# luisdiaz1997/GPzoo

Hardware: AMD Instinct MI355X
Metric: ELBO evals/sec (L=32-latent evaluations, all GPUs) at M=2048 inducing, N=200000, L=32 latents/GPU x 1 GPU(s) (higher is better)
Workload: dtype f32; 1 GPU; BASELINE configs[2]: Slide-seq-shaped synthetic, N=200000 spots, M=2048, L=32 latents/GPU x 1 GPU(s), matern32, f32; latents_total=32, whitened=True, chunk=0, factor_dtype=f64

## Files before the change

### gpzoo_amd/csrc/kgrad.hip

```cpp
#include "kgrad.h"
#include "mmops.h"

namespace gpz {

__device__ __forceinline__ float kg_exp(float x) { return __builtin_amdgcn_exp2f(x * 1.44269504088896341f); }
__device__ __forceinline__ double kg_exp(double x) { return exp(x); }
__device__ __forceinline__ float kg_sqrt(float x) { return sqrtf(x); }
__device__ __forceinline__ double kg_sqrt(double x) { return sqrt(x); }
__device__ __forceinline__ float kg_rsqrt(float x) { return rsqrtf(x); }
__device__ __forceinline__ double kg_rsqrt(double x) { return 1.0 / sqrt(x); }
__device__ __forceinline__ float kg_pow(float x, float y) { return __builtin_amdgcn_exp2f(y * __builtin_amdgcn_logf(x)); }
__device__ __forceinline__ double kg_pow(double x, double y) { return pow(x, y); }

template <typename T, int KIND>
__global__ __launch_bounds__(256) void kgrad_kernel(KgradArgs a) {
  const int l = blockIdx.y, wave = threadIdx.x >> 6, lane = threadIdx.x & 63;
  const int64_t m = (int64_t)blockIdx.x * 4 + wave;
  if (m >= a.M) return;
  const T* kb = static_cast<const T*>(a.Kbar) + (int64_t)l * a.stride + m * a.ld;
  const T* Zp = static_cast<const T*>(a.Z);
  const T* Xp = static_cast<const T*>(a.X);
  const int d = a.d;
  const T sig = static_cast<const T*>(a.sigma)[l];
  const T ell = static_cast<const T*>(a.ell)[l];
  const T s2 = sig * sig, il2 = (T)1 / (ell * ell);
  T z[4] = {0, 0, 0, 0};
  for (int k = 0; k < d; ++k) z[k] = Zp[m * d + k];
  const int gz = (KIND == 2) ? ((uint64_t)a.gZ[m] < (uint64_t)a.G ? (int)a.gZ[m] : 0) : 0;
  const T aeff = (KIND == 2) ? static_cast<const T*>(a.ga)[l] : (T)0;
  const T gpow = (T)a.gpow;
  double dz[4] = {0, 0, 0, 0}, dsig = 0, dell = 0, da = 0;
  constexpr int UN = 4;
  for (int64_t c0 = lane; c0 < a.ncols; c0 += 64 * UN) {
    T g[UN], x[UN][4];
    int gx[UN];
#pragma unroll
    for (int u = 0; u < UN; ++u) {
      const int64_t c = c0 + 64 * u;
      const bool in = c < a.ncols;
      g[u] = in ? kb[c] : (T)0;
#pragma unroll
      for (int k = 0; k < 4; ++k) x[u][k] = (in && k < d) ? Xp[c * d + k] : (T)0;
      gx[u] = (KIND == 2 && in) ? ((uint64_t)a.gX[c] < (uint64_t)a.G ? (int)a.gX[c] : 0) : 0;
    }
    T pz[4] = {0, 0, 0, 0}, psig = 0, pell = 0, pa = 0;
#pragma unroll
    for (int u = 0; u < UN; ++u) {
      T diff[4], d2 = 0;
#pragma unroll
      for (int k = 0; k < 4; ++k) { diff[k] = (k < d) ? z[k] - x[u][k] : (T)0; d2 = fma(diff[k], diff[k], d2); }
      T cz;
      if (KIND == 0) {
        const T kv = s2 * kg_exp((T)-0.5 * d2 * il2);
        psig += g[u] * (T)2 * kv / sig;
        pell += g[u] * kv * d2 * il2 / ell;
        cz = -kv * il2;
      } else if (KIND == 1) {
        const T v = (T)1.7320508075688772935 * kg_sqrt(d2) / ell, e = kg_exp(-v);
        psig += g[u] * (T)2 * sig * ((T)1 + v) * e;
        pell += g[u] * s2 * v * v * e / ell;
        cz = -s2 * (T)3 * il2 * e;
      } else if (KIND == 4) {
        const T rr = kg_sqrt(d2), kv = s2 * kg_exp(-rr / ell);
        psig += g[u] * (T)2 * kv / sig;
        pell += g[u] * kv * rr * il2;
        cz = d2 > (T)0 ? -(kv / ell) * kg_rsqrt(d2) : (T)0;
      } else if (KIND == 5) {
        const T v = (T)2.2360679774997896964 * kg_sqrt(d2) / ell, e = kg_exp(-v), q3 = v * v / (T)3;
        psig += g[u] * (T)2 * sig * ((T)1 + v + q3) * e;
        pell += g[u] * s2 * q3 * ((T)1 + v) * e / ell;
        cz = -s2 * (T)5 / (T)3 * il2 * ((T)1 + v) * e;
      } else {
        const T r2 = static_cast<const T*>(a.gr2)[gz * a.G + gx[u]];
        const T den = aeff * r2 + (T)1;
        const T kv = s2 * kg_exp((T)-0.5 * d2 * il2 / den) * kg_pow(den, -gpow);
        psig += g[u] * (T)2 * kv / sig;
        pell += g[u] * kv * d2 * il2 / (ell * den);
        pa += g[u] * kv * ((T)0.5 * d2 * il2 / (den * den) - gpow / den) * r2;
        cz = -kv * il2 / den;
      }
      const T gc = g[u] * cz;
#pragma unroll
      for (int k = 0; k < 4; ++k) pz[k] = fma(gc, diff[k], pz[k]);
    }
    dsig += (double)psig; dell += (double)pell; da += (double)pa;
#pragma unroll
    for (int k = 0; k < 4; ++k) dz[k] += (double)pz[k];
  }
  double v[7] = {dz[0], dz[1], dz[2], dz[3], dsig * a.scalar_scale, dell * a.scalar_scale, da * a.scalar_scale};
#pragma unroll
  for (int i = 0; i < 7; ++i)
    for (int o = 32; o > 0; o >>= 1) v[i] += __shfl_down(v[i], o);
  if (lane == 0) {
    double* dst = a.acc + ((int64_t)l * a.Mp + m) * 8;
#pragma unroll
    for (int i = 0; i < 7; ++i) dst[i] += v[i];
  }
}

int kgrad_launch(int dtype, int kind, const KgradArgs& a, int L, hipStream_t s) {
  GPZ_REQUIRE((kind >= 0 && kind <= 2) || kind == GPZ_KERNEL_MATERN12 || kind == GPZ_KERNEL_MATERN52,
              "kgrad: unknown kernel kind %d", kind);
  dim3 grid((unsigned)((a.M + 3) / 4), (unsigned)L), block(256);
#define GPZ_KG(T, K) hipLaunchKernelGGL((kgrad_kernel<T, K>), grid, block, 0, s, a)
#define GPZ_KG_KINDS(T) \
  switch (kind) { case 0: GPZ_KG(T, 0); break; case 1: GPZ_KG(T, 1); break; case 4: GPZ_KG(T, 4); break; \
                  case 5: GPZ_KG(T, 5); break; default: GPZ_KG(T, 2); break; }
  if (dtype == GPZ_F32) GPZ_KG_KINDS(float) else GPZ_KG_KINDS(double)
#undef GPZ_KG_KINDS
#undef GPZ_KG
  GPZ_LAUNCH_OK();
  return 0;
}

}

extern "C" size_t gpz_kgrad_workspace_bytes(int64_t nA, int32_t n_latent) {
  if (nA < 1 || n_latent < 1) return 0;
  gpz::Carver c(nullptr);
  c.take<double>((int64_t)n_latent * nA * 8);
  return c.used();
}

extern "C" int gpz_kgrad(const gpz_kernel_desc* k, const void* A, int64_t nA, const void* B, int64_t nB, int32_t d,
                         const int64_t* gA, const int64_t* gB, const void* Kbar, int64_t ldk, int64_t stride_k,
                         double* grad_theta, double* grad_A, void* ws, size_t ws_bytes, void* stream) {
  using namespace gpz;
  GPZ_REQUIRE(k && A && B && Kbar && ws, "gpz_kgrad: null pointer");
  GPZ_REQUIRE(nA >= 1 && nB >= 1 && ldk >= nB && d >= 1 && d <= 4, "gpz_kgrad: bad extents nA=%lld nB=%lld ldk=%lld d=%d",
              (long long)nA, (long long)nB, (long long)ldk, d);
  GPZ_REQUIRE((k->kind >= 0 && k->kind <= 2) || k->kind == GPZ_KERNEL_MATERN12 || k->kind == GPZ_KERNEL_MATERN52,
              "gpz_kgrad: kernel kind %d has no parameters to differentiate", k->kind);
  GPZ_REQUIRE(k->n_latent >= 1 && (k->dtype == GPZ_F32 || k->dtype == GPZ_F64), "gpz_kgrad: bad kernel description");
  if (k->kind == GPZ_KERNEL_MGGP_RBF)
    GPZ_REQUIRE(gA && gB && k->group_a && k->group_r2 && k->n_groups >= 1, "gpz_kgrad: MGGP kernel needs groups, group_a, group_r2");
  GPZ_REQUIRE(ws_bytes >= gpz_kgrad_workspace_bytes(nA, k->n_latent), "gpz_kgrad: workspace too small");
  hipStream_t s = static_cast<hipStream_t>(stream);
  const int L = k->n_latent;
  Carver c(ws);
  double* acc = c.take<double>((int64_t)L * nA * 8);
  GPZ_HIP_OK(hipMemsetAsync(acc, 0, sizeof(double) * L * nA * 8, s));
  KgradArgs a;
  a.Kbar = Kbar; a.ld = ldk; a.stride = stride_k; a.Z = A; a.X = B; a.gZ = gA; a.gX = gB;
  a.sigma = k->sigma; a.ell = k->lengthscale; a.ga = k->group_a; a.gr2 = k->group_r2;
  a.gpow = k->group_pow; a.scalar_scale = 1.0; a.M = nA; a.ncols = nB; a.Mp = nA; a.d = d; a.G = k->n_groups; a.acc = acc;
  if (int rc = kgrad_launch(k->dtype, k->kind, a, L, s)) return rc;
  return kgrad_finish(acc, L, nA, nA, d, nullptr, grad_A, grad_theta, s);
}
```

Baseline: 2.654 ELBO evals/s.

## Restructure kgrad kernel: two rows per wave, factored sums, vector loads, templated dim

Each wavefront now handles two inducing rows and reuses every loaded X column for both. Columns are read as 4-wide vector loads, and the input dimension becomes a template parameter. The per-element math is rewritten to accumulate a few kernel-specific moment sums (e, e*r, e*d2, ...) with sigma, lengthscale and constants folded into the exponent scale, and the gradients are rebuilt in double once per row at the end. This is meant to cut redundant X loads, per-element divides and multiplies, and wasted lanes when d<4. In exchange it adds register pressure and many more template instantiations, and the vector loads assume 16-byte-friendly alignment of Kbar rows.

```diff
diff --git a/gpzoo_amd/csrc/kgrad.hip b/gpzoo_amd/csrc/kgrad.hip
--- a/gpzoo_amd/csrc/kgrad.hip
+++ b/gpzoo_amd/csrc/kgrad.hip
@@ -3,111 +3,216 @@
 
 namespace gpz {
 
-__device__ __forceinline__ float kg_exp(float x) { return __builtin_amdgcn_exp2f(x * 1.44269504088896341f); }
-__device__ __forceinline__ double kg_exp(double x) { return exp(x); }
-__device__ __forceinline__ float kg_sqrt(float x) { return sqrtf(x); }
-__device__ __forceinline__ double kg_sqrt(double x) { return sqrt(x); }
-__device__ __forceinline__ float kg_rsqrt(float x) { return rsqrtf(x); }
-__device__ __forceinline__ double kg_rsqrt(double x) { return 1.0 / sqrt(x); }
-__device__ __forceinline__ float kg_pow(float x, float y) { return __builtin_amdgcn_exp2f(y * __builtin_amdgcn_logf(x)); }
-__device__ __forceinline__ double kg_pow(double x, double y) { return pow(x, y); }
-
-template <typename T, int KIND>
+constexpr int KG_ROWS = 2;
+
+template <typename T> struct KgMath;
+template <> struct KgMath<float> {
+  typedef float vec4 __attribute__((ext_vector_type(4), aligned(4)));
+  static constexpr float escale = 1.44269504088896341f;
+  static __device__ __forceinline__ float exps(float x) { return __builtin_amdgcn_exp2f(x); }
+  static __device__ __forceinline__ float sqrt(float x) { return __builtin_amdgcn_sqrtf(x); }
+  static __device__ __forceinline__ float rsqrt(float x) { return rsqrtf(x); }
+  static __device__ __forceinline__ float rcp(float x) { return __builtin_amdgcn_rcpf(x); }
+  static __device__ __forceinline__ float pow(float x, float y) { return __builtin_amdgcn_exp2f(y * __builtin_amdgcn_logf(x)); }
+};
+template <> struct KgMath<double> {
+  typedef double vec4 __attribute__((ext_vector_type(4), aligned(8)));
+  static constexpr double escale = 1.0;
+  static __device__ __forceinline__ double exps(double x) { return ::exp(x); }
+  static __device__ __forceinline__ double sqrt(double x) { return ::sqrt(x); }
+  static __device__ __forceinline__ double rsqrt(double x) { return 1.0 / ::sqrt(x); }
+  static __device__ __forceinline__ double rcp(double x) { return 1.0 / x; }
+  static __device__ __forceinline__ double pow(double x, double y) { return ::pow(x, y); }
+};
+
+__host__ __device__ constexpr int kg_nsums(int kind) { return kind == 0 ? 2 : kind == 1 ? 3 : kind == 4 ? 2 : 4; }
+
+template <typename T> struct KgConst { T c2, c1, aeff, gpow; };
+
+template <typename T, bool FULL>
+__device__ __forceinline__ void kg_load4(const T* p, int64_t c, int64_t n, T (&o)[4]) {
+  if (FULL) {
+    const typename KgMath<T>::vec4 q = *reinterpret_cast<const typename KgMath<T>::vec4*>(p + c);
+    o[0] = q.x; o[1] = q.y; o[2] = q.z; o[3] = q.w;
+  } else {
+#pragma unroll
+    for (int j = 0; j < 4; ++j) o[j] = c + j < n ? p[c + j] : (T)0;
+  }
+}
+
+template <typename T, int D, int R> struct KgTrip { T g[R][4], x[4 * D]; int gx[4]; };
+
+template <typename T, int KIND, int D, int R, bool FULL>
+__device__ __forceinline__ void kg_load(const KgradArgs& a, const T* (&kb)[R], const T* Xp, int64_t c,
+                                        KgTrip<T, D, R>& t) {
+#pragma unroll
+  for (int r = 0; r < R; ++r) kg_load4<T, FULL>(kb[r], c, a.ncols, t.g[r]);
+#pragma unroll
+  for (int q = 0; q < D; ++q) {
+    T o[4];
+    kg_load4<T, FULL>(Xp, c * D + 4 * q, a.ncols * D, o);
+#pragma unroll
+    for (int j = 0; j < 4; ++j) t.x[4 * q + j] = o[j];
+  }
+#pragma unroll
+  for (int j = 0; j < 4; ++j)
+    t.gx[j] = (KIND == 2 && (FULL || c + j < a.ncols)) ? ((uint64_t)a.gX[c + j] < (uint64_t)a.G ? (int)a.gX[c + j] : 0) : 0;
+}
+
+template <typename T, int KIND, int D, int R>
+__device__ __forceinline__ void kg_accum(const KgradArgs& a, const KgConst<T>& k, const T (&z)[R][D], const int (&gz)[R],
+                                         const KgTrip<T, D, R>& t, T (&S)[R][kg_nsums(KIND) + D]) {
+  using Mth = KgMath<T>;
+  constexpr int NS = kg_nsums(KIND);
+#pragma unroll
+  for (int j = 0; j < 4; ++j)
+#pragma unroll
+    for (int r = 0; r < R; ++r) {
+      T diff[D];
+      diff[0] = z[r][0] - t.x[j * D];
+      T d2 = diff[0] * diff[0];
+#pragma unroll
+      for (int q = 1; q < D; ++q) { diff[q] = z[r][q] - t.x[j * D + q]; d2 = fma(diff[q], diff[q], d2); }
+      const T g = t.g[r][j];
+      T w;
+      if (KIND == 0) {
+        const T e = g * Mth::exps(d2 * k.c2);
+        S[r][0] += e; S[r][1] = fma(e, d2, S[r][1]);
+        w = e;
+      } else if (KIND == 1) {
+        const T rr = Mth::sqrt(d2), e = g * Mth::exps(rr * k.c2);
+        S[r][0] += e; S[r][1] = fma(e, rr, S[r][1]); S[r][2] = fma(e, d2, S[r][2]);
+        w = e;
+      } else if (KIND == 4) {
+        const T ri = d2 > (T)0 ? Mth::rsqrt(d2) : (T)0, rr = d2 * ri, e = g * Mth::exps(rr * k.c2);
+        S[r][0] += e; S[r][1] = fma(e, rr, S[r][1]);
+        w = e * ri;
+      } else if (KIND == 5) {
+        const T rr = Mth::sqrt(d2), e = g * Mth::exps(rr * k.c2), er = e * rr;
+        S[r][0] += e; S[r][1] += er; S[r][2] = fma(e, d2, S[r][2]); S[r][3] = fma(er, d2, S[r][3]);
+        w = fma(er, k.c1, e);
+      } else {
+        const T r2 = static_cast<const T*>(a.gr2)[gz[r] * a.G + t.gx[j]];
+        const T den = fma(k.aeff, r2, (T)1), id = Mth::rcp(den);
+        const T e = g * Mth::exps(d2 * k.c2 * id) * Mth::pow(den, -k.gpow), u = e * id, ur = u * r2;
+        S[r][0] += e; S[r][1] = fma(u, d2, S[r][1]); S[r][2] = fma(ur * id, d2, S[r][2]); S[r][3] += ur;
+        w = u;
+      }
+#pragma unroll
+      for (int q = 0; q < D; ++q) S[r][NS + q] = fma(w, diff[q], S[r][NS + q]);
+    }
+}
+
+template <int KIND, int D>
+__device__ __forceinline__ void kg_finish_row(const double* v, double sig, double ell, double gpow, double scale, double* dst) {
+  constexpr int NS = kg_nsums(KIND);
+  const double il = 1.0 / ell, s2 = sig * sig, il2 = il * il;
+  double dsig, dell, da = 0, fz;
+  if (KIND == 0) {
+    dsig = 2 * sig * v[0]; dell = s2 * il2 * il * v[1]; fz = -s2 * il2;
+  } else if (KIND == 1) {
+    const double c1 = 1.7320508075688772935 * il;
+    dsig = 2 * sig * (v[0] + c1 * v[1]); dell = s2 * il * c1 * c1 * v[2]; fz = -3 * s2 * il2;
+  } else if (KIND == 4) {
+    dsig = 2 * sig * v[0]; dell = s2 * il2 * v[1]; fz = -s2 * il;
+  } else if (KIND == 5) {
+    const double c1 = 2.2360679774997896964 * il, q = c1 * c1 / 3;
+    dsig = 2 * sig * (v[0] + c1 * v[1] + q * v[2]); dell = s2 * il * q * (v[2] + c1 * v[3]); fz = -(5.0 / 3.0) * s2 * il2;
+  } else {
+    dsig = 2 * sig * v[0]; dell = s2 * il2 * il * v[1]; da = s2 * (0.5 * il2 * v[2] - gpow * v[3]); fz = -s2 * il2;
+  }
+#pragma unroll
+  for (int q = 0; q < D; ++q) dst[q] += fz * v[NS + q];
+  dst[4] += dsig * scale; dst[5] += dell * scale;
+  if (KIND == 2) dst[6] += da * scale;
+}
+
+template <typename T, int KIND, int D>
 __global__ __launch_bounds__(256) void kgrad_kernel(KgradArgs a) {
+  constexpr int R = KG_ROWS, NS = kg_nsums(KIND), NV = NS + D;
+  using Mth = KgMath<T>;
   const int l = blockIdx.y, wave = threadIdx.x >> 6, lane = threadIdx.x & 63;
-  const int64_t m = (int64_t)blockIdx.x * 4 + wave;
-  if (m >= a.M) return;
-  const T* kb = static_cast<const T*>(a.Kbar) + (int64_t)l * a.stride + m * a.ld;
+  const int64_t m0 = ((int64_t)blockIdx.x * 4 + wave) * R;
+  if (m0 >= a.M) return;
   const T* Zp = static_cast<const T*>(a.Z);
   const T* Xp = static_cast<const T*>(a.X);
-  const int d = a.d;
+  const T* kbl = static_cast<const T*>(a.Kbar) + (int64_t)l * a.stride;
   const T sig = static_cast<const T*>(a.sigma)[l];
   const T ell = static_cast<const T*>(a.ell)[l];
-  const T s2 = sig * sig, il2 = (T)1 / (ell * ell);
-  T z[4] = {0, 0, 0, 0};
-  for (int k = 0; k < d; ++k) z[k] = Zp[m * d + k];
-  const int gz = (KIND == 2) ? ((uint64_t)a.gZ[m] < (uint64_t)a.G ? (int)a.gZ[m] : 0) : 0;
-  const T aeff = (KIND == 2) ? static_cast<const T*>(a.ga)[l] : (T)0;
-  const T gpow = (T)a.gpow;
-  double dz[4] = {0, 0, 0, 0}, dsig = 0, dell = 0, da = 0;
-  constexpr int UN = 4;
-  for (int64_t c0 = lane; c0 < a.ncols; c0 += 64 * UN) {
-    T g[UN], x[UN][4];
-    int gx[UN];
-#pragma unroll
-    for (int u = 0; u < UN; ++u) {
-      const int64_t c = c0 + 64 * u;
-      const bool in = c < a.ncols;
-      g[u] = in ? kb[c] : (T)0;
-#pragma unroll
-      for (int k = 0; k < 4; ++k) x[u][k] = (in && k < d) ? Xp[c * d + k] : (T)0;
-      gx[u] = (KIND == 2 && in) ? ((uint64_t)a.gX[c] < (uint64_t)a.G ? (int)a.gX[c] : 0) : 0;
-    }
-    T pz[4] = {0, 0, 0, 0}, psig = 0, pell = 0, pa = 0;
-#pragma unroll
-    for (int u = 0; u < UN; ++u) {
-      T diff[4], d2 = 0;
-#pragma unroll
-      for (int k = 0; k < 4; ++k) { diff[k] = (k < d) ? z[k] - x[u][k] : (T)0; d2 = fma(diff[k], diff[k], d2); }
-      T cz;
-      if (KIND == 0) {
-        const T kv = s2 * kg_exp((T)-0.5 * d2 * il2);
-        psig += g[u] * (T)2 * kv / sig;
-        pell += g[u] * kv * d2 * il2 / ell;
-        cz = -kv * il2;
-      } else if (KIND == 1) {
-        const T v = (T)1.7320508075688772935 * kg_sqrt(d2) / ell, e = kg_exp(-v);
-        psig += g[u] * (T)2 * sig * ((T)1 + v) * e;
-        pell += g[u] * s2 * v * v * e / ell;
-        cz = -s2 * (T)3 * il2 * e;
-      } else if (KIND == 4) {
-        const T rr = kg_sqrt(d2), kv = s2 * kg_exp(-rr / ell);
-        psig += g[u] * (T)2 * kv / sig;
-        pell += g[u] * kv * rr * il2;
-        cz = d2 > (T)0 ? -(kv / ell) * kg_rsqrt(d2) : (T)0;
-      } else if (KIND == 5) {
-        const T v = (T)2.2360679774997896964 * kg_sqrt(d2) / ell, e = kg_exp(-v), q3 = v * v / (T)3;
-        psig += g[u] * (T)2 * sig * ((T)1 + v + q3) * e;
-        pell += g[u] * s2 * q3 * ((T)1 + v) * e / ell;
-        cz = -s2 * (T)5 / (T)3 * il2 * ((T)1 + v) * e;
-      } else {
-        const T r2 = static_cast<const T*>(a.gr2)[gz * a.G + gx[u]];
-        const T den = aeff * r2 + (T)1;
-        const T kv = s2 * kg_exp((T)-0.5 * d2 * il2 / den) * kg_pow(den, -gpow);
-        psig += g[u] * (T)2 * kv / sig;
-        pell += g[u] * kv * d2 * il2 / (ell * den);
-        pa += g[u] * kv * ((T)0.5 * d2 * il2 / (den * den) - gpow / den) * r2;
-        cz = -kv * il2 / den;
-      }
-      const T gc = g[u] * cz;
-#pragma unroll
-      for (int k = 0; k < 4; ++k) pz[k] = fma(gc, diff[k], pz[k]);
-    }
-    dsig += (double)psig; dell += (double)pell; da += (double)pa;
-#pragma unroll
-    for (int k = 0; k < 4; ++k) dz[k] += (double)pz[k];
-  }
-  double v[7] = {dz[0], dz[1], dz[2], dz[3], dsig * a.scalar_scale, dell * a.scalar_scale, da * a.scalar_scale};
-#pragma unroll
-  for (int i = 0; i < 7; ++i)
-    for (int o = 32; o > 0; o >>= 1) v[i] += __shfl_down(v[i], o);
+  const T il = (T)1 / ell;
+  KgConst<T> k;
+  k.c1 = (T)2.2360679774997896964 * il;
+  k.c2 = (KIND == 1 ? (T)-1.7320508075688772935 * il : KIND == 4 ? -il : KIND == 5 ? -k.c1 : (T)-0.5 * il * il) * Mth::escale;
+  k.aeff = (KIND == 2) ? static_cast<const T*>(a.ga)[l] : (T)0;
+  k.gpow = (T)a.gpow;
+  const T* kb[R];
+  T z[R][D];
+  int gz[R];
+#pragma unroll
+  for (int r = 0; r < R; ++r) {
+    const int64_t m = m0 + r < a.M ? m0 + r : a.M - 1;
+    kb[r] = kbl + m * a.ld;
+#pragma unroll
+    for (int q = 0; q < D; ++q) z[r][q] = Zp[m * D + q];
+    gz[r] = (KIND == 2) ? ((uint64_t)a.gZ[m] < (uint64_t)a.G ? (int)a.gZ[m] : 0) : 0;
+  }
+  T S[R][NV];
+  double tot[R][NV];
+#pragma unroll
+  for (int r = 0; r < R; ++r)
+#pragma unroll
+    for (int i = 0; i < NV; ++i) { S[r][i] = 0; tot[r][i] = 0; }
+  auto fold = [&]() {
+#pragma unroll
+    for (int r = 0; r < R; ++r)
+#pragma unroll
+      for (int i = 0; i < NV; ++i) { tot[r][i] += (double)S[r][i]; S[r][i] = 0; }
+  };
+  const int64_t nfull = a.ncols / 512;
+  for (int64_t it = 0; it < nfull; ++it) {
+    const int64_t c = it * 512 + lane * 4;
+    KgTrip<T, D, R> t0, t1;
+    kg_load<T, KIND, D, R, true>(a, kb, Xp, c, t0);
+    kg_load<T, KIND, D, R, true>(a, kb, Xp, c + 256, t1);
+    kg_accum<T, KIND, D, R>(a, k, z, gz, t0, S);
+    kg_accum<T, KIND, D, R>(a, k, z, gz, t1, S);
+    fold();
+  }
+  for (int64_t c0 = nfull * 512; c0 < a.ncols; c0 += 256) {
+    KgTrip<T, D, R> t;
+    kg_load<T, KIND, D, R, false>(a, kb, Xp, c0 + lane * 4, t);
+    kg_accum<T, KIND, D, R>(a, k, z, gz, t, S);
+  }
+  fold();
+#pragma unroll
+  for (int r = 0; r < R; ++r)
+#pragma unroll
+    for (int i = 0; i < NV; ++i)
+      for (int o = 32; o > 0; o >>= 1) tot[r][i] += __shfl_down(tot[r][i], o);
   if (lane == 0) {
-    double* dst = a.acc + ((int64_t)l * a.Mp + m) * 8;
-#pragma unroll
-    for (int i = 0; i < 7; ++i) dst[i] += v[i];
+#pragma unroll
+    for (int r = 0; r < R; ++r)
+      if (m0 + r < a.M)
+        kg_finish_row<KIND, D>(tot[r], (double)sig, (double)ell, a.gpow, a.scalar_scale,
+                               a.acc + ((int64_t)l * a.Mp + m0 + r) * 8);
   }
 }
 
 int kgrad_launch(int dtype, int kind, const KgradArgs& a, int L, hipStream_t s) {
   GPZ_REQUIRE((kind >= 0 && kind <= 2) || kind == GPZ_KERNEL_MATERN12 || kind == GPZ_KERNEL_MATERN52,
               "kgrad: unknown kernel kind %d", kind);
-  dim3 grid((unsigned)((a.M + 3) / 4), (unsigned)L), block(256);
-#define GPZ_KG(T, K) hipLaunchKernelGGL((kgrad_kernel<T, K>), grid, block, 0, s, a)
+  GPZ_REQUIRE(a.d >= 1 && a.d <= 4, "kgrad: input dimension %d outside 1..4", a.d);
+  dim3 grid((unsigned)((a.M + 4 * KG_ROWS - 1) / (4 * KG_ROWS)), (unsigned)L), block(256);
+#define GPZ_KG(T, K, D) hipLaunchKernelGGL((kgrad_kernel<T, K, D>), grid, block, 0, s, a)
+#define GPZ_KG_DIMS(T, K) \
+  switch (a.d) { case 1: GPZ_KG(T, K, 1); break; case 2: GPZ_KG(T, K, 2); break; case 3: GPZ_KG(T, K, 3); break; \
+                 default: GPZ_KG(T, K, 4); break; }
 #define GPZ_KG_KINDS(T) \
-  switch (kind) { case 0: GPZ_KG(T, 0); break; case 1: GPZ_KG(T, 1); break; case 4: GPZ_KG(T, 4); break; \
-                  case 5: GPZ_KG(T, 5); break; default: GPZ_KG(T, 2); break; }
+  switch (kind) { case 0: GPZ_KG_DIMS(T, 0) break; case 1: GPZ_KG_DIMS(T, 1) break; case 4: GPZ_KG_DIMS(T, 4) break; \
+                  case 5: GPZ_KG_DIMS(T, 5) break; default: GPZ_KG_DIMS(T, 2) break; }
   if (dtype == GPZ_F32) GPZ_KG_KINDS(float) else GPZ_KG_KINDS(double)
 #undef GPZ_KG_KINDS
+#undef GPZ_KG_DIMS
 #undef GPZ_KG
   GPZ_LAUNCH_OK();
   return 0;
```

Result: no change. 2.648 ELBO evals/s (-0.2%).
